# ethanabrooks/hsr-env

Measured on NVIDIA B200. Metric: env_actions_per_sec, higher is better.
Workload: dtype f32

## Files before the change

### hsr_env_b200/csrc/hsr_core.h

```cpp
#pragma once
#include <cfloat>
#include <cmath>
#include <cstdint>

#include "hsr_model.h"

#if defined(__CUDACC__)
#define HSR_HD __host__ __device__ __forceinline__
#define HSR_HDN __host__ __device__ __noinline__
#if defined(HSR_COMPACT)
#define HSR_HDC __host__ __device__ __noinline__
#else
#define HSR_HDC __host__ __device__ __forceinline__
#endif
#else
#define HSR_HDC inline
#define HSR_HD inline
#define HSR_HDN inline
#endif

#if defined(HSR_SCAN_NOISE) && !defined(__CUDA_ARCH__)
static thread_local unsigned long long hsr_scan_noise_seed = 0;
#endif

// ... 489 lines not shown
  st3(r, cross(va, fa) + cross(vl, fl)); st3(r + 3, cross(va, fl));
}

template <typename T>
HSR_HDC void smooth_lane0(const ModelT<T>& m, WS<T>& w) {
  int nv = m.nv;
  T (*cvel)[6] = reinterpret_cast<T(*)[6]>(w.cvel);
  T (*cacc)[6] = reinterpret_cast<T(*)[6]>(w.cacc);
  T (*cfrc)[6] = reinterpret_cast<T(*)[6]>(w.cfrc);
  for (int k = 0; k < 6; k++) { cvel[0][k] = 0; cacc[0][k] = 0; cfrc[0][k] = 0; }
  cacc[0][3] = -m.gravity[0]; cacc[0][4] = -m.gravity[1]; cacc[0][5] = -m.gravity[2];
  for (int b = 1; b < m.nbody; b++) {
    int p = m.body_parent[b];
    T v[6], a[6], t[6];
    for (int k = 0; k < 6; k++) { v[k] = cvel[p][k]; a[k] = cacc[p][k]; }
    for (int j = m.body_jntadr[b]; j < m.body_jntadr[b] + m.body_jntnum[b]; j++) {
      int d0 = m.jnt_dofadr[j];
      if (m.jnt_type[j] == JNT_FREE) {
        for (int k = 0; k < 3; k++) for (int i = 0; i < 6; i++) v[i] += w.cdof[6 * (d0 + k) + i] * w.qvel[d0 + k];
        T vt[6];
        for (int i = 0; i < 6; i++) vt[i] = v[i];
        for (int k = 3; k < 6; k++) {
          cross_motion(vt, w.cdof + 6 * (d0 + k), t);
          for (int i = 0; i < 6; i++) { a[i] += t[i] * w.qvel[d0 + k]; v[i] += w.cdof[6 * (d0 + k) + i] * w.qvel[d0 + k]; }
        }
      } else {
        cross_motion(v, w.cdof + 6 * d0, t);
        for (int i = 0; i < 6; i++) { a[i] += t[i] * w.qvel[d0]; v[i] += w.cdof[6 * d0 + i] * w.qvel[d0]; }
      }
    }
    T Ia[6], Iv[6];
    inert_mul(w.binert + 10 * b, a, Ia);
    inert_mul(w.binert + 10 * b, v, Iv);
    cross_force(v, Iv, t);
    for (int k = 0; k < 6; k++) { cvel[b][k] = v[k]; cacc[b][k] = a[k]; cfrc[b][k] = Ia[k] + t[k]; }
  }
  for (int b = m.nbody - 1; b > 0; b--) {
    int p = m.body_parent[b];
    if (p > 0) for (int k = 0; k < 6; k++) cfrc[p][k] += cfrc[b][k];
  }
  for (int i = 0; i < nv; i++) {
    const T* c = w.cdof + 6 * i;
    const T* f = cfrc[m.dof_body[i]];
    T bias = c[0] * f[0] + c[1] * f[1] + c[2] * f[2] + c[3] * f[3] + c[4] * f[4] + c[5] * f[5];
    w.qfrc_smooth[i] = -m.dof_damping[i] * w.qvel[i] - bias;
  }
  for (int a = 0; a < m.nu; a++) {
    T c = w.ctrl[a];
    if (m.act_ctrllimited[a]) c = fmin(fmax(c, m.act_ctrlrange[2 * a]), m.act_ctrlrange[2 * a + 1]);
    T f = m.act_kp[a] * c - m.act_kp[a] * m.act_gear[a] * w.qpos[m.act_qposadr[a]];
    if (m.act_forcelimited[a]) f = fmin(fmax(f, m.act_forcerange[2 * a]), m.act_forcerange[2 * a + 1]);
    w.qfrc_smooth[m.act_dof[a]] += m.act_gear[a] * f;
  }
}
template <typename T, typename Grp>
HSR_HD void smooth_solve(const ModelT<T>& m, WS<T>& w, const Grp& g) {
  const int nv = m.nv;
  for (int k = g.lane; k < nv * nv; k += Grp::G) w.L[k] = w.M[k];
  for (int i = g.lane; i < nv; i += Grp::G) w.qacc_smooth[i] = w.qfrc_smooth[i];
  g.sync();
  if (!chol_factor_g(w.L, nv, w.invd, g) && g.lane == 0) w.wi[WI_FLAGS] |= FLAG_CHOL;
  chol_solve_g(w.L, nv, w.invd, w.qacc_smooth, g);
}

template <typename T> struct Geom {
  int type; T size[3]; const T* verts; int nvert; V3<GT> pos; GT mat[9];
  const T* verts4 = nullptr;
};

template <typename T>
HSR_HD void load_geom(const ModelT<T>& m, const WS<T>& w, int gi, Geom<T>& ge) {
  ge.type = m.geom_type[gi];
  for (int k = 0; k < 3; k++) ge.size[k] = m.geom_size[3 * gi + k];
  ge.verts = m.hull_vert + 3 * m.geom_vertadr[gi]; ge.nvert = m.geom_vertnum[gi];
  ge.pos = ld3(w.gpos + 3 * gi);
  GT gm[9];
  for (int k = 0; k < 9; k++) gm[k] = (GT)m.geom_mat[9 * gi + k];
  mulm(w.xmat + 9 * m.geom_body[gi], gm, ge.mat);
}

template <typename T> HSR_HD void make_frame(V3<GT> n, T* fr) {
  n = normalized(n);
  V3<GT> t = (n.y > GT(-0.5) && n.y < GT(0.5)) ? mk<GT>(0, 1, 0) : mk<GT>(0, 0, 1);
  t = t - n * dot(n, t);
  t = normalized(t);
  st3c(fr, n); st3c(fr + 3, t); st3c(fr + 6, cross(n, t));
}

template <typename T, typename Grp>
HSR_HDC void add_contact(const ModelT<T>& m, WS<T>& w, const Grp& g, int& ncon, int& nrow, int pair, GT dist, V3<GT> pos,
                        V3<GT> n) {
  int dim = m.pair_condim[pair];
  if (ncon >= m.ncon_max || nrow + dim > m.nefc_max) {
    if (g.lane == 0) w.wi[WI_FLAGS] |= FLAG_CON_OVERFLOW;
    return;
  }
  if (g.lane == 0) {
    w.con_pair[ncon] = pair; w.con_dist[ncon] = (T)dist; st3c(w.con_pos + 3 * ncon, pos);
    make_frame(n, w.con_frame + 9 * ncon);
    w.con_adr[ncon] = nrow;
  }
  ncon++; nrow += dim;
}

template <typename T> struct Sup { V3<T> v, v1, v2; };

template <typename T> HSR_HD bool is_zero(T x) { return fabs(x) < Lim<T>::eps(); }
template <typename T> HSR_HD bool ccd_eq(T a, T b) {
  T ab = fabs(a - b);
  if (ab < Lim<T>::eps()) return true;
  a = fabs(a); b = fabs(b);
  return ab < Lim<T>::eps() * (b > a ? b : a);
}

template <typename T> HSR_HD T origin_tri_dist2(V3<T> a, V3<T> b, V3<T> c, V3<T>& q) {
  V3<T> ab = b - a, ac = c - a, ap = -a;
  T d1 = dot(ab, ap), d2 = dot(ac, ap);
  if (d1 <= 0 && d2 <= 0) { q = a; return dot(q, q); }
  V3<T> bp = -b;
  T d3 = dot(ab, bp), d4 = dot(ac, bp);
  if (d3 >= 0 && d4 <= d3) { q = b; return dot(q, q); }
  T vc = d1 * d4 - d3 * d2;
  V3<T> cp = -c;
  T d5 = dot(ab, cp), d6 = dot(ac, cp);
  if (vc <= 0 && d1 >= 0 && d3 <= 0) { q = a + ab * (d1 / (d1 - d3)); return dot(q, q); }
  if (d6 >= 0 && d5 <= d6) { q = c; return dot(q, q); }
  T vb = d5 * d2 - d1 * d6, va = d3 * d6 - d5 * d4;
  if (vb <= 0 && d2 >= 0 && d6 <= 0) { q = a + ac * (d2 / (d2 - d6)); return dot(q, q); }
  if (va <= 0 && (d4 - d3) >= 0 && (d5 - d6) >= 0) { q = b + (c - b) * ((d4 - d3) / ((d4 - d3) + (d5 - d6))); return dot(q, q); }
  T den = T(1) / (va + vb + vc);
  q = a + ab * (vb * den) + ac * (vc * den);
  return dot(q, q);
}

#define HSR_SUPPORT_TIE 1e-12
template <typename T> HSR_HD T scan_slack(T best) { return sizeof(T) == 4 ? T(1e-6) * (T(1) + fabs(best)) : T(HSR_SUPPORT_TIE); }
HSR_HD double dot3_exact(double x, double y, double z, double lx, double ly, double lz) {
#if defined(__CUDA_ARCH__)
  return __dadd_rn(__dadd_rn(__dmul_rn(x, lx), __dmul_rn(y, ly)), __dmul_rn(z, lz));
#else
  volatile double a = x * lx, b = y * ly, c = z * lz;
  volatile double ab = a + b;
  return ab + c;
#endif
}

template <typename T> HSR_HD void load_vert(const T* p, int st, T& x, T& y, T& z) { (void)st; x = p[0]; y = p[1]; z = p[2]; }
#if defined(__CUDACC__)
template <> HSR_HD void load_vert<float>(const float* p, int st, float& x, float& y, float& z) {
  if (st == 4) { const float4 a = *reinterpret_cast<const float4*>(p); x = a.x; y = a.y; z = a.z; }
  else { x = p[0]; y = p[1]; z = p[2]; }
}
#endif
template <typename T, typename Grp>
HSR_HD int hull_argmax(const T* __restrict__ v, int st, int n, V3<double> dl, const Grp& g) {
  const T lx = (T)dl.x, ly = (T)dl.y, lz = (T)dl.z;
  T best = -FLT_MAX, second = -FLT_MAX;
  int bi = 0x7fffffff;
  for (int i = g.lane; i < n; i += Grp::G) {
    T px, py, pz;
    load_vert(v + (size_t)st * i, st, px, py, pz);
    T val = px * lx + py * ly + pz * lz;
#if defined(HSR_SCAN_NOISE) && !defined(__CUDA_ARCH__)
    if (hsr_scan_noise_seed) {
      hsr_scan_noise_seed = hsr_scan_noise_seed * 6364136223846793005ull + 1442695040888963407ull;
      val += (T)(fabs((double)val) * 2.4e-7 * ((double)(hsr_scan_noise_seed >> 40) / 16777216.0 - 0.5));
    }
#endif
    if (val > best) bi = i;
    second = fmax(second, fmin(best, val));
    best = fmax(best, val);
  }
  T gbest = best;
  int gbi = bi;
  g.argmax(gbest, gbi);
  const T cut = gbest - scan_slack(gbest);
  const unsigned involved = g.ballot(best >= cut);
  const unsigned multi = g.ballot(second >= cut);
  if (multi == 0 && (involved & (involved - 1)) == 0) return gbi;
  if (multi == 0) {
    double dv = -DBL_MAX;
    if (best >= cut) {
      T px, py, pz;
      load_vert(v + (size_t)st * bi, st, px, py, pz);
      dv = dot3_exact((double)px, (double)py, (double)pz, dl.x, dl.y, dl.z);
    }
    const double dmax = g.max(dv);
    return g.min(dv >= dmax - HSR_SUPPORT_TIE ? bi : 0x7fffffff);
  }
  double dbest = -DBL_MAX;
  if (best >= cut) {
    for (int i = g.lane; i < n; i += Grp::G) {
      T px, py, pz;
      load_vert(v + (size_t)st * i, st, px, py, pz);
      const T val = px * lx + py * ly + pz * lz;
      if (val >= cut) { const double d = dot3_exact((double)px, (double)py, (double)pz, dl.x, dl.y, dl.z); if (d > dbest) dbest = d; }
    }
  }
  dbest = g.max(dbest);
  int mi = 0x7fffffff;
  if (best >= cut) {
    for (int i = g.lane; i < n; i += Grp::G) {
      T px, py, pz;
      load_vert(v + (size_t)st * i, st, px, py, pz);
      const T val = px * lx + py * ly + pz * lz;
      if (val >= cut && i < mi && dot3_exact((double)px, (double)py, (double)pz, dl.x, dl.y, dl.z) >= dbest - HSR_SUPPORT_TIE) mi = i;
    }
  }
  return g.min(mi);
}

template <typename T, typename Grp>
HSR_HD V3<double> support_d(const Geom<T>& ge, V3<double> d, const Grp& g) {
  typedef double W;
  const W* R = ge.mat;
  V3<W> dl = multv(R, d), res;
  const W tie = -HSR_SUPPORT_TIE;
  if (ge.type == GEOM_BOX) {
    res = mk<W>(dl.x >= tie ? (W)ge.size[0] : -(W)ge.size[0], dl.y >= tie ? (W)ge.size[1] : -(W)ge.size[1],
                dl.z >= tie ? (W)ge.size[2] : -(W)ge.size[2]);
  } else if (ge.type == GEOM_CYLINDER) {
    W n = sqrt(dl.x * dl.x + dl.y * dl.y);
    res = mk<W>(0, 0, dl.z >= tie ? (W)ge.size[1] : -(W)ge.size[1]);
    if (n > 1e-15) { res.x = dl.x / n * (W)ge.size[0]; res.y = dl.y / n * (W)ge.size[0]; }
#if defined(__CUDACC__)
  } else if (ge.verts4) {
    const int bi = hull_argmax<float>(ge.verts4, 4, ge.nvert, dl, g);
    res = mk<W>((W)ge.verts4[4 * bi], (W)ge.verts4[4 * bi + 1], (W)ge.verts4[4 * bi + 2]);
#endif
  } else {
    const int bi = hull_argmax<T>(ge.verts, 3, ge.nvert, dl, g);
    res = mk<W>((W)ge.verts[3 * bi], (W)ge.verts[3 * bi + 1], (W)ge.verts[3 * bi + 2]);
  }
  return ge.pos + mulv(R, res);
}

template <typename T, typename Grp>
HSR_HD void mpr_support(const Geom<T>& g1, const Geom<T>& g2, V3<double> d, const Grp& g, Sup<double>& s) {
  s.v1 = support_d(g1, d, g); s.v2 = support_d(g2, -d, g); s.v = s.v1 - s.v2;
}

template <typename T, typename Grp>
HSR_HD bool mpr_penetration_inl(const Geom<T>& g1, const Geom<T>& g2, GT tol, int max_iter, const Grp& g, GT& depth_,
                                V3<GT>& pdir_, V3<GT>& ppos_, float* sep = nullptr);
template <typename T, typename Grp>
HSR_HDN bool mpr_penetration(const Geom<T>& g1, const Geom<T>& g2, GT tol, int max_iter, const Grp& g, GT& depth_,
                             V3<GT>& pdir_, V3<GT>& ppos_, float* sep = nullptr) {
  return mpr_penetration_inl(g1, g2, tol, max_iter, g, depth_, pdir_, ppos_, sep);
}
template <typename T, typename Grp>
HSR_HD bool mpr_penetration_inl(const Geom<T>& g1, const Geom<T>& g2, GT tol, int max_iter, const Grp& g, GT& depth_,
                                V3<GT>& pdir_, V3<GT>& ppos_, float* sep) {
  typedef double W;
  auto sup = [&](V3<W> d) { Sup<W> s; mpr_support(g1, g2, d, g, s); return s; };
  auto miss = [&](V3<W> d) {
    if (sep && g.lane == 0) { sep[0] = (float)d.x; sep[1] = (float)d.y; sep[2] = (float)d.z; sep[3] = 1.f; }
    return false;
  };
  if (sep && sep[3] == 1.f) {
    V3<W> dc = normalized(mk<W>((W)sep[0], (W)sep[1], (W)sep[2]));
    Sup<W> sc = sup(dc);
    W dtc = dot(sc.v, dc);
    if (dtc < 0 && !is_zero(dtc)) return false;
    g.sync();
    if (g.lane == 0) sep[3] = 0.f;
  }
  auto reach_tol = [&](const Sup<W>& v1, const Sup<W>& v2, const Sup<W>& v3, const Sup<W>& v4, V3<W> d) {
    W dv4 = dot(v4.v, d);
    W d1 = dv4 - dot(v1.v, d), d2 = dv4 - dot(v2.v, d), d3 = dv4 - dot(v3.v, d);
    W mn = fmin(d1, fmin(d2, d3));
    return ccd_eq(mn, tol) || mn < tol;
  };
  auto expand = [&](const Sup<W>& v0, Sup<W>& v1, Sup<W>& v2, Sup<W>& v3, const Sup<W>& v4) {
    V3<W> v4v0 = cross(v4.v, v0.v);
    if (dot(v1.v, v4v0) > 0) {
      if (dot(v2.v, v4v0) > 0) v1 = v4; else v3 = v4;
    } else {
      if (dot(v3.v, v4v0) > 0) v2 = v4; else v1 = v4;
    }
  };
  auto finish = [&](W depth, V3<W> dir, V3<W> pos) {
    depth_ = depth; pdir_ = dir; ppos_ = pos;
    if (sep && g.lane == 0) sep[3] = 2.f;
    return true;
  };
  const W eps = Lim<W>::eps();
  Sup<W> v0, v1, v2, v3, v4;
  v0.v1 = g1.pos; v0.v2 = g2.pos;
  v0.v = v0.v1 - v0.v2;
  if (fabs(v0.v.x) < eps && fabs(v0.v.y) < eps && fabs(v0.v.z) < eps) v0.v.x += eps * 10;
  V3<W> d = normalized(-v0.v);
  v1 = sup(d);
  W dt = dot(v1.v, d);
  if (is_zero(dt) || dt < 0) return dt < 0 && !is_zero(dt) ? miss(d) : false;
  d = cross(v0.v, v1.v);
  if (is_zero(dot(d, d))) {
    if (fabs(v1.v.x) < eps && fabs(v1.v.y) < eps && fabs(v1.v.z) < eps) return false;
    W dep = norm(v1.v);
    return finish(dep, v1.v * (W(1) / dep), (v1.v1 + v1.v2) * W(0.5));
  }
  d = normalized(d);
  v2 = sup(d);
  dt = dot(v2.v, d);
  if (is_zero(dt) || dt < 0) return dt < 0 && !is_zero(dt) ? miss(d) : false;
  d = normalized(cross(v1.v - v0.v, v2.v - v0.v));
  if (dot(d, v0.v) > 0) { Sup<W> t = v1; v1 = v2; v2 = t; d = -d; }
  for (int guard = 0; guard < 64; guard++) {
    v3 = sup(d);
    dt = dot(v3.v, d);
    if (is_zero(dt) || dt < 0) return dt < 0 && !is_zero(dt) ? miss(d) : false;
    bool cont = false;
    dt = dot(cross(v1.v, v3.v), v0.v);
    if (dt < 0 && !is_zero(dt)) { v2 = v3; cont = true; }
    if (!cont) {
      dt = dot(cross(v3.v, v2.v), v0.v);
      if (dt < 0 && !is_zero(dt)) { v1 = v3; cont = true; }
    }
    if (!cont) break;
    d = normalized(cross(v1.v - v0.v, v2.v - v0.v));
  }
  for (int guard = 0; guard < 256; guard++) {
    d = normalized(cross(v2.v - v1.v, v3.v - v1.v));
    dt = dot(d, v1.v);
    if (is_zero(dt) || dt > 0) break;
    v4 = sup(d);
    dt = dot(v4.v, d);
    if (!(is_zero(dt) || dt > 0)) return miss(d);
    if (reach_tol(v1, v2, v3, v4, d)) return false;
    expand(v0, v1, v2, v3, v4);
  }
  int it = 0;
  while (true) {
    d = normalized(cross(v2.v - v1.v, v3.v - v1.v));
    v4 = sup(d);
    if (reach_tol(v1, v2, v3, v4, d) || it > max_iter) {
      V3<W> q;
      W d2 = origin_tri_dist2(v1.v, v2.v, v3.v, q);
      W dep = sqrt(d2);
      if (is_zero(dep)) return false;
      V3<W> dir = q * (W(1) / norm(q));
      W b0 = dot(cross(v1.v, v2.v), v3.v), b1 = dot(cross(v3.v, v2.v), v0.v), b2 = dot(cross(v0.v, v1.v), v3.v),
        b3 = dot(cross(v2.v, v1.v), v0.v);
      W s = b0 + b1 + b2 + b3;
      if (is_zero(s) || s < 0) {
        b0 = 0; b1 = dot(cross(v2.v, v3.v), d); b2 = dot(cross(v3.v, v1.v), d); b3 = dot(cross(v1.v, v2.v), d);
        s = b1 + b2 + b3;
      }
      W inv = W(1) / s;
      V3<W> p1 = (v0.v1 * b0 + v1.v1 * b1 + v2.v1 * b2 + v3.v1 * b3) * inv;
      V3<W> p2 = (v0.v2 * b0 + v1.v2 * b1 + v2.v2 * b2 + v3.v2 * b3) * inv;
      return finish(dep, dir, (p1 + p2) * W(0.5));
    }
    expand(v0, v1, v2, v3, v4);
    it++;
  }
}

template <typename T, typename Grp>
HSR_HDN void box_box(const ModelT<T>& m, WS<T>& w, const Grp& g, int& ncon, int& nrow, int pair, const Geom<T>& A,
                     const Geom<T>& B) {
  const GT* R1 = A.mat; const GT* R2 = B.mat;
  const GT s1[3] = {(GT)A.size[0], (GT)A.size[1], (GT)A.size[2]}, s2[3] = {(GT)B.size[0], (GT)B.size[1], (GT)B.size[2]};
// ... 876 lines not shown
```

### hsr_env_b200/csrc/hsrb_wpe.cuh

```cuda
#pragma once
#include "hsrb_push.cuh"

#ifndef WPE_MAXCON
#define WPE_MAXCON 8
#endif
#define WPE_GROUPS (WPE_MAXCON + 2)
#define WPE_SLOTS (6 * WPE_GROUPS)
#define WPE_MAXROW (6 * WPE_MAXCON + 2)
#define WPE_MAXBG 2
#define WPE_MAXGEOM 24
#define WPE_MAXPAIR 24
#define WPE_ENVJOBS 7
#ifndef WPE_MAXWARPS
#define WPE_MAXWARPS 28
#endif

namespace wpe {

struct alignas(16) Tab {
  double gbase[WPE_MAXGEOM * 3];
  double gmatw[WPE_MAXGEOM * 9];
  double pairc[WPE_MAXPAIR * PUSH_PAIRC];
  float ghalf[WPE_MAXGEOM * 3];
  float geom_rbound[WPE_MAXGEOM];
  float geom_size[WPE_MAXGEOM * 3];
  float pair_friction[WPE_MAXPAIR * 5];
  float bgeom_mat[WPE_MAXBG * 9];
  float geom_aabb[WPE_MAXGEOM * 3];
  int gmove[WPE_MAXGEOM], geom_type[WPE_MAXGEOM], geom_vertadr[WPE_MAXGEOM], geom_vertnum[WPE_MAXGEOM];
  int pair_geom1[WPE_MAXPAIR], pair_geom2[WPE_MAXPAIR], pair_func[WPE_MAXPAIR], pair_condim[WPE_MAXPAIR];
  float pair_sr[WPE_MAXPAIR], pair_sb[WPE_MAXPAIR];
  int gb0;
  float blk_radius;
  int wpt;
  unsigned char team[WPE_MAXWARPS];
};

struct alignas(16) Slice {
  double xb[4], Rb[10], bmat[9 * WPE_MAXBG], gpos[WPE_MAXGEOM * 3], portal[48], mres[8];
  float qpos[12], qvel[8], warm[8], mocap[4], ctrl[4];
  float baabb[4 * WPE_MAXBG];
  float qs[8], as[8], x[8], qfc[8], srch[8];
  float con_dist[WPE_MAXCON], con_pos[WPE_MAXCON * 3], con_frame[WPE_MAXCON * 9];
  int con_pair[WPE_MAXCON], con_adr[WPE_MAXCON], wi[4];
  int acc[8];
  float jres[WPE_ENVJOBS * 14 + 2];
  float J[WPE_SLOTS * 8];
  float Dr[WPE_SLOTS], aref[WPE_SLOTS], rsc[WPE_SLOTS], jar[WPE_SLOTS], jv[WPE_SLOTS], f[WPE_SLOTS], wrow[WPE_SLOTS];
  float PQ[16 * WPE_GROUPS], wpq[2 * WPE_GROUPS + 4], L[64];
  float sep[4 * WPE_MAXPAIR];
};

#define WPE_MAXTEAMS 4
struct alignas(16) Queue {
  int cnt[WPE_MAXTEAMS][4];
  int jobs[WPE_MAXWARPS * WPE_ENVJOBS];
};

static_assert(offsetof(Slice, J) % 16 == 0 && offsetof(Slice, PQ) % 16 == 0 && offsetof(Slice, L) % 16 == 0 && offsetof(Slice, qpos) % 16 == 0 &&
              offsetof(Slice, qvel) % 16 == 0 && offsetof(Slice, qs) % 16 == 0 && offsetof(Slice, x) % 16 == 0 && offsetof(Slice, srch) % 16 == 0 &&
              offsetof(Slice, warm) % 16 == 0 && offsetof(Slice, as) % 16 == 0 && sizeof(Slice) % 16 == 0,
              "128-bit shared-memory accesses (push::ld8 / st8) need 16-byte aligned fields");
__host__ __device__ inline size_t slice_bytes() { return sizeof(Slice); }
constexpr unsigned SMEM_HEAD = (unsigned)(sizeof(Tab) + sizeof(Queue));
static_assert(SMEM_HEAD % 16 == 0, "the slices start 16-byte aligned");
__host__ __device__ inline size_t shared_tail(const ModelT<float>& m) { return SMEM_HEAD + (size_t)m.nvert * 16 + 16; }

}

#if defined(HSRB_WPE_IMPL)
namespace wpe {

typedef V3<double> V3d;

__device__ __forceinline__ unsigned char* smem_base() {
  HSRB_DYN_SMEM(smem);
  return smem;
}
__device__ __forceinline__ Tab& tab() { return *reinterpret_cast<Tab*>(smem_base()); }
__device__ __forceinline__ Queue& queue() { return *reinterpret_cast<Queue*>(smem_base() + sizeof(Tab)); }
__device__ __forceinline__ Slice& slice(int w) { return *reinterpret_cast<Slice*>(smem_base() + SMEM_HEAD + (unsigned)w * (unsigned)sizeof(Slice)); }
__device__ __forceinline__ float* hull_verts4() {
  return reinterpret_cast<float*>(smem_base() + SMEM_HEAD + (blockDim.x >> 5) * (unsigned)sizeof(Slice));
}

#if defined(WPE_CHAIN_CLOCKS)
__device__ unsigned long long wpe_ck_cyc[32], wpe_ck_cnt[32];
#define WPE_CK_DECL long long ck_last = clock64()
#define WPE_CK_RESET() do { ck_last = clock64(); } while (0)
#define WPE_CK(id) do { if ((threadIdx.x & 31) == 0) { const long long t_ = clock64(); atomicAdd(&wpe::wpe_ck_cyc[id], (unsigned long long)(t_ - ck_last)); atomicAdd(&wpe::wpe_ck_cnt[id], 1ull); } ck_last = clock64(); } while (0)
#else
#define WPE_CK_DECL do { } while (0)
#define WPE_CK_RESET() do { } while (0)
#define WPE_CK(id) do { } while (0)
#endif

#if defined(HSRB_SIMT_EMU)
__device__ __forceinline__ void team_sync(int team, int nthreads) { emu::named_barrier(1 + team, nthreads); }
__device__ __forceinline__ bool team_and(int team, int nthreads, bool p) { return emu::named_vote(1 + team, nthreads, p, true); }
#else
__device__ __forceinline__ void team_sync(int team, int nthreads) {
  asm volatile("bar.sync %0, %1;" ::"r"(1 + team), "r"(nthreads) : "memory");
}
__device__ __forceinline__ bool team_and(int team, int nthreads, bool p) {
  unsigned r;
  asm volatile(
      "{\n\t.reg .pred q, r;\n\tsetp.ne.u32 q, %3, 0;\n\tbar.red.and.pred r, %1, %2, q;\n\tselp.u32 %0, 1, 0, r;\n\t}"
      : "=r"(r) : "r"(1 + team), "r"(nthreads), "r"((unsigned)p) : "memory");
  return r != 0;
}
#endif

__device__ __forceinline__ float warp_sum(float v) {
#pragma unroll
  for (int o = 16; o > 0; o >>= 1) v += __shfl_xor_sync(0xffffffffu, v, o);
  return v;
}

__device__ __forceinline__ const double* geom_mat(const Tab& t, const Slice& s, int gi, int gb0) {
  return t.gmove[gi] == 2 ? s.bmat + 9 * (gi - gb0) : t.gmatw + 9 * gi;
}

#ifndef WPE_SUPPORT_ATTR
#define WPE_SUPPORT_ATTR __forceinline__
#endif
__device__ WPE_SUPPORT_ATTR V3d support(const Tab& t, const Slice& s, const float* verts4, int gi, int gb0, V3d d) {
  WPE_CK_DECL;
  const double* R = geom_mat(t, s, gi, gb0);
  const V3d dl = multv(R, d);
  const int type = t.geom_type[gi];
  const float* sz = t.geom_size + 3 * gi;
  V3d res;
  const double tie = -HSR_SUPPORT_TIE;
  if (type == GEOM_BOX) {
    res = mk<double>(dl.x >= tie ? (double)sz[0] : -(double)sz[0], dl.y >= tie ? (double)sz[1] : -(double)sz[1],
                     dl.z >= tie ? (double)sz[2] : -(double)sz[2]);
  } else if (type == GEOM_CYLINDER) {
    const double n = sqrt(dl.x * dl.x + dl.y * dl.y);
    res = mk<double>(0, 0, dl.z >= tie ? (double)sz[1] : -(double)sz[1]);
    if (n > 1e-15) { res.x = dl.x / n * (double)sz[0]; res.y = dl.y / n * (double)sz[0]; }
  } else {
    const DevGrp<32> gw;
    const float* v4 = verts4 + 4 * t.geom_vertadr[gi];
    WPE_CK(22);
    const int bi = hull_argmax<float>(v4, 4, t.geom_vertnum[gi], dl, gw);
    WPE_CK(23);
    res = mk<double>((double)v4[4 * bi], (double)v4[4 * bi + 1], (double)v4[4 * bi + 2]);
  }
  const V3d out_ = ld3(s.gpos + 3 * gi) + mulv(R, res);
  WPE_CK(type == GEOM_BOX ? 25 : 24);
  return out_;
}

__device__ __forceinline__ V3d pv(const Slice& s, int k) { return ld3(s.portal + 9 * k); }
__device__ __forceinline__ void pcopy(Slice& s, int dst, int src) {
  const int lane = threadIdx.x & 31;
  __syncwarp();
  if (lane < 9) s.portal[9 * dst + lane] = s.portal[9 * src + lane];
  __syncwarp();
}

__device__ __noinline__ bool mpr(int ow, int g1, int g2, int gb0, float tol_f, int max_iter, int sepk) {
  const Tab& t = tab();
  const Slice& o = slice(ow);
  Slice& s = slice(threadIdx.x >> 5);
  const float* const verts4 = hull_verts4();
  float* const sep = sepk >= 0 ? slice(ow).sep + 4 * sepk : nullptr;
  const double tol = (double)tol_f;
  double* const out7 = s.mres;
  double* const P = s.portal;
  const int lane = threadIdx.x & 31;
  enum { S_CACHE = 0, S_V1, S_V2, S_DISCOVER, S_REFINE, S_PENETRATE };
  const double eps = DBL_EPSILON;
  int state = S_V1;
  V3d dcur;
  {
    V3d v0 = ld3(o.gpos + 3 * g1) - ld3(o.gpos + 3 * g2);
    if (fabs(v0.x) < eps && fabs(v0.y) < eps && fabs(v0.z) < eps) v0.x += eps * 10;
    V3d d;
    if (sep && (sep[3] == 1.f || sep[3] < 0.f)) {
      state = S_CACHE;
      d = normalized(mk<double>((double)sep[0], (double)sep[1], (double)sep[2]));
    } else {
      d = normalized(-v0);
    }
    __syncwarp();
    if (lane == 0) { st3(P, v0); st3(P + 3, ld3(o.gpos + 3 * g1)); st3(P + 6, ld3(o.gpos + 3 * g2)); }
    __syncwarp();
    dcur = d;
  }
  int guard = 0, it = 0;
  WPE_CK_DECL;
#define WPE_NEXT_DIR() { dcur = d; WPE_CK(21); continue; }
#pragma unroll 1
  while (true) {
    const V3d a1 = support(t, o, verts4, g1, gb0, dcur);
    const V3d a2 = support(t, o, verts4, g2, gb0, -dcur);
    const V3d v4 = a1 - a2;
    __syncwarp();
    if (lane == 0) { st3(P + 36, v4); st3(P + 39, a1); st3(P + 42, a2); }
    WPE_CK(20);
    V3d d = dcur;
    const V3d v0 = ld3(P);
    double dt = dot(v4, d);
    bool enter_refine = false;
    if (state == S_CACHE) {
      if (dt < 0 && !is_zero(dt)) {
        if (lane == 0) sep[3] = (float)(dt * 0.999);
        return false;
      }
      if (lane == 0) sep[3] = 0.f;
      state = S_V1;
      d = normalized(-v0);
      WPE_NEXT_DIR();
    }
    if (state <= S_DISCOVER) {
      if (is_zero(dt) || dt < 0) {
        if (dt < 0 && !is_zero(dt) && sep && lane == 0) { sep[0] = (float)d.x; sep[1] = (float)d.y; sep[2] = (float)d.z; sep[3] = (float)(dt * 0.999); }
        return false;
      }
    }
    if (state == S_V1) {
      pcopy(s, 1, 4);
      d = cross(v0, v4);
      if (is_zero(dot(d, d))) {
        if (fabs(v4.x) < eps && fabs(v4.y) < eps && fabs(v4.z) < eps) return false;
        const double dep = norm(v4);
        const V3d dir = v4 * (1.0 / dep), pos = (a1 + a2) * 0.5;
        if (lane == 0) {
          out7[0] = dep; out7[1] = dir.x; out7[2] = dir.y; out7[3] = dir.z; out7[4] = pos.x; out7[5] = pos.y; out7[6] = pos.z;
          if (sep) sep[3] = 2.f;
        }
        __syncwarp();
        return true;
      }
      d = normalized(d);
      state = S_V2;
      WPE_NEXT_DIR();
    }
    if (state == S_V2) {
      pcopy(s, 2, 4);
      const V3d v1 = pv(s, 1);
      d = normalized(cross(v1 - v0, v4 - v0));
      if (dot(d, v0) > 0) {
        pcopy(s, 2, 1); pcopy(s, 1, 4);
        d = -d;
      }
      state = S_DISCOVER; guard = 0;
      WPE_NEXT_DIR();
    }
    if (state == S_DISCOVER) {
      pcopy(s, 3, 4);
      const V3d v1 = pv(s, 1), v2 = pv(s, 2);
      bool cont = false;
      dt = dot(cross(v1, v4), v0);
      if (dt < 0 && !is_zero(dt)) { pcopy(s, 2, 3); cont = true; }
      if (!cont) {
        dt = dot(cross(v4, v2), v0);
        if (dt < 0 && !is_zero(dt)) { pcopy(s, 1, 3); cont = true; }
      }
      guard++;
      if (cont && guard < 64) {
        const V3d w1 = pv(s, 1), w2 = pv(s, 2);
        d = normalized(cross(w1 - v0, w2 - v0));
        WPE_NEXT_DIR();
      }
      state = S_REFINE; guard = 0;
      enter_refine = true;
    }
    if (state == S_REFINE && !enter_refine) {
      if (!(is_zero(dt) || dt > 0)) {
        if (sep && lane == 0) { sep[0] = (float)d.x; sep[1] = (float)d.y; sep[2] = (float)d.z; sep[3] = (float)(dt * 0.999); }
        return false;
      }
    }
    if (state == S_PENETRATE || (state == S_REFINE && !enter_refine)) {
      const V3d v1 = pv(s, 1), v2 = pv(s, 2), v3 = pv(s, 3);
      const double d1 = dt - dot(v1, d), d2 = dt - dot(v2, d), d3 = dt - dot(v3, d);
      const double mn = fmin(d1, fmin(d2, d3));
      const bool reach = ccd_eq(mn, tol) || mn < tol;
      if (state == S_REFINE) {
        if (reach) return false;
      } else if (reach || it > max_iter) {
        V3d q;
        const double dd2 = origin_tri_dist2(v1, v2, v3, q);
        const double dep = sqrt(dd2);
        if (is_zero(dep)) return false;
        const V3d dir = q * (1.0 / norm(q));
        double b0 = dot(cross(v1, v2), v3), b1 = dot(cross(v3, v2), v0), b2 = dot(cross(v0, v1), v3), b3 = dot(cross(v2, v1), v0);
        double sm = b0 + b1 + b2 + b3;
        if (is_zero(sm) || sm < 0) {
          b0 = 0; b1 = dot(cross(v2, v3), d); b2 = dot(cross(v3, v1), d); b3 = dot(cross(v1, v2), d);
          sm = b1 + b2 + b3;
        }
        const double inv = 1.0 / sm;
        const double* P = s.portal;
        const V3d p1 = (ld3(P + 3) * b0 + ld3(P + 12) * b1 + ld3(P + 21) * b2 + ld3(P + 30) * b3) * inv;
        const V3d p2 = (ld3(P + 6) * b0 + ld3(P + 15) * b1 + ld3(P + 24) * b2 + ld3(P + 33) * b3) * inv;
        const V3d pos = (p1 + p2) * 0.5;
        if (lane == 0) {
          out7[0] = dep; out7[1] = dir.x; out7[2] = dir.y; out7[3] = dir.z; out7[4] = pos.x; out7[5] = pos.y; out7[6] = pos.z;
          if (sep) sep[3] = 2.f;
        }
        __syncwarp();
        return true;
      }
      const V3d v4v0 = cross(v4, v0);
      int repl;
      if (dot(v1, v4v0) > 0) repl = dot(v2, v4v0) > 0 ? 1 : 3;
      else repl = dot(v3, v4v0) > 0 ? 2 : 1;
      pcopy(s, repl, 4);
      if (state == S_REFINE) guard++; else it++;
    }
    {
      const V3d v1 = pv(s, 1), v2 = pv(s, 2), v3 = pv(s, 3);
      d = normalized(cross(v2 - v1, v3 - v1));
      if (state == S_REFINE) {
        const double dv = dot(d, v1);
        if (is_zero(dv) || dv > 0 || guard >= 256) state = S_PENETRATE;
      }
    }
    WPE_NEXT_DIR();
  }
#undef WPE_NEXT_DIR
}

__device__ __forceinline__ int* team_jobs(Queue& Q, const Tab& t, int w) { return Q.jobs + t.team[w] * t.wpt * WPE_ENVJOBS; }

}

#if defined(HSRB_PHASE_CLOCKS)
#define WPE_PH(id) do { if (LOCK && threadIdx.x == 0) { const long long t_ = clock64(); ph[id] += (unsigned long long)(t_ - tlast) >> 4; tlast = t_; } } while (0)
#else
#define WPE_PH(id) do { } while (0)
#endif
template <bool LOCK>
__global__ void __launch_bounds__(32 * WPE_MAXWARPS, 1) hsrb_wpe_kernel_t(const __grid_constant__ KArgs a, const __grid_constant__ PushInfo fi) {
  constexpr unsigned FULL = 0xffffffffu;
  const int lane = threadIdx.x & 31, wib = threadIdx.x >> 5, wpb = blockDim.x >> 5;
  const ModelT<float>& m = a.m;
  wpe::Tab& tw = wpe::tab();
  wpe::Queue& Q = wpe::queue();
  float* const v4w = wpe::hull_verts4();
  {
    const int ng = m.ngeom, np = m.npair;
    for (int i = threadIdx.x; i < m.nvert * 4; i += blockDim.x) v4w[i] = fi.verts4[i];
#define TAB_COPY(field, src, n) for (int i = threadIdx.x; i < (n); i += blockDim.x) tw.field[i] = (src)[i];
    TAB_COPY(gbase, fi.gbase, ng * 3) TAB_COPY(gmatw, fi.gmatw, ng * 9) TAB_COPY(pairc, fi.pairc, np * PUSH_PAIRC)
    TAB_COPY(ghalf, fi.ghalf, ng * 3) TAB_COPY(geom_rbound, m.geom_rbound, ng)
    TAB_COPY(geom_size, m.geom_size, ng * 3) TAB_COPY(pair_friction, m.pair_friction, np * 5)
    TAB_COPY(geom_aabb, m.geom_aabb, ng * 3)
    {
      int gb0_ = ng;
      for (int i = ng - 1; i >= 0; i--) if (fi.gmove[i] == 2) gb0_ = i;
      for (int i = threadIdx.x; i < (ng - gb0_) * 9 && i < WPE_MAXBG * 9; i += blockDim.x) tw.bgeom_mat[i] = m.geom_mat[9 * gb0_ + i];
      if (threadIdx.x == 0) {
        float blk_radius = 0.f;
        for (int i = gb0_; i < ng; i++) {
          const double* o3 = fi.gbase + 3 * i;
          blk_radius = fmaxf(blk_radius, (float)sqrt(o3[0] * o3[0] + o3[1] * o3[1] + o3[2] * o3[2]) * 1.001f + m.geom_rbound[i]);
        }
        tw.gb0 = gb0_; tw.blk_radius = blk_radius;
      }
      int nteam = LOCK ? (int)((a.opts >> 4) & 15u) : 1;
      if (nteam < 1 || nteam > WPE_MAXTEAMS || wpb % nteam != 0) nteam = 1;
      if (threadIdx.x == 0) tw.wpt = wpb / nteam;
      if (threadIdx.x < wpb) tw.team[threadIdx.x] = (unsigned char)(threadIdx.x / (wpb / nteam));
    }
    TAB_COPY(gmove, fi.gmove, ng) TAB_COPY(geom_type, m.geom_type, ng)
    TAB_COPY(geom_vertadr, m.geom_vertadr, ng) TAB_COPY(geom_vertnum, m.geom_vertnum, ng)
    TAB_COPY(pair_geom1, m.pair_geom1, np) TAB_COPY(pair_geom2, m.pair_geom2, np)
    TAB_COPY(pair_func, m.pair_func, np) TAB_COPY(pair_condim, m.pair_condim, np)
#undef TAB_COPY
    for (int k = threadIdx.x; k < np; k += blockDim.x) {
      const int b1 = m.geom_body[m.pair_geom1[k]], b2 = m.geom_body[m.pair_geom2[k]];
      tw.pair_sr[k] = (float)(b2 == fi.robot_body) - (float)(b1 == fi.robot_body);
      tw.pair_sb[k] = (float)(b2 == fi.block_body) - (float)(b1 == fi.block_body);
    }
    if (threadIdx.x < 4 * WPE_MAXTEAMS) (&Q.cnt[0][0])[threadIdx.x] = 0;
    __syncthreads();
  }
  const wpe::Tab& t = tw;
  const float* const verts4 = v4w;
  wpe::Slice& s = wpe::slice(wib);
  const int NV = fi.nv;
  const bool HASB = NV == 8;
  const int nq = m.nq;
  const float dt = m.timestep;
  const int li = lane & 7, sub = lane >> 3;
  const float scale = 1.0f / (m.meaninertia * (float)(NV > 1 ? NV : 1));
  const float Mi = li < NV ? fi.Mdiag[li] : 1.0f, dampi = li < NV ? fi.damp[li] : 0.f;
  const bool use_sep = !(a.opts & 1u);
  const bool use_gap = use_sep && !(a.opts & 0x10000u);
#if !defined(HSRB_SIMT_EMU)
  if (LOCK && t.team[wib] > 0 && ((a.opts >> 8) & 255u)) {
    const long long t0 = clock64(), wait = (long long)((a.opts >> 8) & 255u) * 4 * 1965 * t.team[wib];
    while (clock64() - t0 < wait) __nanosleep(1000);
  }
#endif
#if defined(WPE_DEBUG_JOBS)
  long long dbg_long = 0, dbg_quick = 0; int dbg_nlong = 0, dbg_nquick = 0, dbg_hits = 0, dbg_jobs_total = 0, dbg_long_total = 0, dbg_sub = 0;
#endif
#if defined(HSRB_PHASE_CLOCKS)
  unsigned long long ph[PH_COUNT] = {0, 0, 0, 0, 0, 0, 0};
  long long tlast = clock64();
#endif

#pragma unroll 1
  for (int wave0 = 0; wave0 < a.n; wave0 += gridDim.x * wpb) {
    const int slot = wave0 + wib * (int)gridDim.x + (int)blockIdx.x;
    const bool valid = slot < a.n;
    const int env = valid ? (a.order ? a.order[slot] : slot) : 0;
    if (!LOCK && !valid) break;
    if (valid) {
      const float* st = a.state + (size_t)env * a.S;
      if (lane < 12) s.qpos[lane] = (lane < nq) ? st[lane] : 0.f;
      if (lane < 8) {
        s.qvel[lane] = lane < NV ? st[nq + lane] : 0.f;
        s.warm[lane] = lane < NV ? st[nq + NV + lane] : 0.f;
        s.qfc[lane] = 0.f;
      }
      if (lane < 3) s.mocap[lane] = st[nq + 2 * NV + lane];
      if (lane < 2) s.ctrl[lane] = (a.ctrl && lane < fi.act_n) ? a.ctrl[(size_t)env * m.nu + lane] : 0.f;
      if (lane < 4) s.wi[lane] = 0;
      for (int i = lane; i < 4 * m.npair; i += 32) s.sep[i] = 0.f;
      for (int i = lane; i < m.ngeom * 3; i += 32) s.gpos[i] = t.gbase[i];
      if (lane < 3) s.xb[lane] = 0;
      if (lane < 9) s.Rb[lane] = (lane % 4 == 0) ? 1.0 : 0.0;
    }
    int flags = 0;
    enum { A_ITER = 0, A_LS, A_CON, A_EFC, A_KFLOP, A_NARROW, A_HIT };
    if (lane < 8) s.acc[lane] = 0;
#if defined(WPE_CHAIN_CLOCKS)
    const long long ck_env0 = clock64();
#endif
    bool success = false;
    int taken = 0;
    bool finished = !valid || a.nsub <= 0;
    __syncwarp();

#pragma unroll 1
    for (int sb_ = 0; sb_ < a.nsub; sb_++) {
      if (LOCK) { if (wpe::team_and(t.team[wib], 32 * t.wpt, finished)) break; }
      else if (finished) break;
#if defined(HSRB_PHASE_CLOCKS)
      if (LOCK && threadIdx.x == 0) tlast = clock64();
#endif
      int nlimit = 0, ncon = 0, nefc = 0, narrow = 0, npflop = 0, ngrp = 0, nslot = 0, gdim = 0, nskip = 0;
      unsigned bits = 0;
      int it = 0, ls_used = 0;
      WPE_CK_DECL;
      if (!finished) {
      if (HASB) {
        double qd[4] = {(double)s.qpos[5], (double)s.qpos[6], (double)s.qpos[7], (double)s.qpos[8]};
        quatnormalize(qd);
        double Rb[9];
        quat2mat(qd, Rb);
        __syncwarp();
        if (lane < 4) s.qpos[5 + lane] = (float)qd[lane];
        if (lane < 3) s.xb[lane] = (double)s.qpos[2 + lane];
        if (lane == 0) {
#pragma unroll
          for (int k = 0; k < 9; k++) s.Rb[k] = Rb[k];
        }
// ... 791 lines not shown
```

Baseline: 216,600.

## Unroll hull support scan and keep MPR portal candidate in registers

Splits hull_argmax into a scan phase and a pick phase. The scan can now keep U independent running maxima so vertex loads can overlap, with U set to 2 for the warp-per-env path. The MPR portal's candidate point (v4, a1, a2) is no longer written to shared slot 4. Each of lanes 0-8 holds one component in a register and writes it straight into its destination slot, which shrinks the shared Slice portal array and removes a store plus a sync. The sep pointer becomes a lazily evaluated lambda, and the extra unrolled accumulators cost registers.

```diff
diff --git a/hsr_env_b200/csrc/hsr_core.h b/hsr_env_b200/csrc/hsr_core.h
--- a/hsr_env_b200/csrc/hsr_core.h
+++ b/hsr_env_b200/csrc/hsr_core.h
@@ -665,25 +665,47 @@
   else { x = p[0]; y = p[1]; z = p[2]; }
 }
 #endif
-template <typename T, typename Grp>
-HSR_HD int hull_argmax(const T* __restrict__ v, int st, int n, V3<double> dl, const Grp& g) {
+template <typename T> struct HullScan { T best, second; int bi; };
+template <int U, typename T, typename Grp>
+HSR_HD HullScan<T> hull_scan(const T* __restrict__ v, int st, int n, V3<double> dl, const Grp& g) {
   const T lx = (T)dl.x, ly = (T)dl.y, lz = (T)dl.z;
-  T best = -FLT_MAX, second = -FLT_MAX;
-  int bi = 0x7fffffff;
-  for (int i = g.lane; i < n; i += Grp::G) {
-    T px, py, pz;
-    load_vert(v + (size_t)st * i, st, px, py, pz);
-    T val = px * lx + py * ly + pz * lz;
+  HullScan<T> a[U];
+#pragma unroll
+  for (int u = 0; u < U; u++) { a[u].best = -FLT_MAX; a[u].second = -FLT_MAX; a[u].bi = 0x7fffffff; }
+  for (int i0 = g.lane; i0 < n; i0 += U * Grp::G) {
+#pragma unroll
+    for (int u = 0; u < U; u++) {
+      const int i = i0 + u * Grp::G;
+      const bool in = u == 0 || i < n;
+      T px, py, pz;
+      load_vert(v + (size_t)st * (in ? i : i0), st, px, py, pz);
+      T val = px * lx + py * ly + pz * lz;
 #if defined(HSR_SCAN_NOISE) && !defined(__CUDA_ARCH__)
-    if (hsr_scan_noise_seed) {
-      hsr_scan_noise_seed = hsr_scan_noise_seed * 6364136223846793005ull + 1442695040888963407ull;
-      val += (T)(fabs((double)val) * 2.4e-7 * ((double)(hsr_scan_noise_seed >> 40) / 16777216.0 - 0.5));
-    }
+      if (hsr_scan_noise_seed && in) {
+        hsr_scan_noise_seed = hsr_scan_noise_seed * 6364136223846793005ull + 1442695040888963407ull;
+        val += (T)(fabs((double)val) * 2.4e-7 * ((double)(hsr_scan_noise_seed >> 40) / 16777216.0 - 0.5));
+      }
 #endif
-    if (val > best) bi = i;
-    second = fmax(second, fmin(best, val));
-    best = fmax(best, val);
-  }
+      if (!in) val = -FLT_MAX;
+      if (val > a[u].best) a[u].bi = i;
+      a[u].second = fmax(a[u].second, fmin(a[u].best, val));
+      a[u].best = fmax(a[u].best, val);
+    }
+  }
+#pragma unroll
+  for (int u = 1; u < U; u++) {
+    if (a[u].best > a[0].best || (a[u].best == a[0].best && a[u].bi < a[0].bi)) a[0].bi = a[u].bi;
+    a[0].second = fmax(fmax(a[0].second, a[u].second), fmin(a[0].best, a[u].best));
+    a[0].best = fmax(a[0].best, a[u].best);
+  }
+  return a[0];
+}
+
+template <typename T, typename Grp>
+HSR_HD int hull_pick(const T* __restrict__ v, int st, int n, V3<double> dl, const Grp& g, const HullScan<T>& sc) {
+  const T lx = (T)dl.x, ly = (T)dl.y, lz = (T)dl.z;
+  const T best = sc.best, second = sc.second;
+  const int bi = sc.bi;
   T gbest = best;
   int gbi = bi;
   g.argmax(gbest, gbi);
@@ -721,6 +743,11 @@
     }
   }
   return g.min(mi);
+}
+
+template <typename T, typename Grp>
+HSR_HD int hull_argmax(const T* __restrict__ v, int st, int n, V3<double> dl, const Grp& g) {
+  return hull_pick(v, st, n, dl, g, hull_scan<1>(v, st, n, dl, g));
 }
 
 template <typename T, typename Grp>
diff --git a/hsr_env_b200/csrc/hsrb_wpe.cuh b/hsr_env_b200/csrc/hsrb_wpe.cuh
--- a/hsr_env_b200/csrc/hsrb_wpe.cuh
+++ b/hsr_env_b200/csrc/hsrb_wpe.cuh
@@ -37,7 +37,7 @@
 };
 
 struct alignas(16) Slice {
-  double xb[4], Rb[10], bmat[9 * WPE_MAXBG], gpos[WPE_MAXGEOM * 3], portal[48], mres[8];
+  double xb[4], Rb[10], bmat[9 * WPE_MAXBG], gpos[WPE_MAXGEOM * 3], portal[36], mres[8];
   float qpos[12], qvel[8], warm[8], mocap[4], ctrl[4];
   float baabb[4 * WPE_MAXBG];
   float qs[8], as[8], x[8], qfc[8], srch[8];
@@ -121,6 +121,9 @@
   return t.gmove[gi] == 2 ? s.bmat + 9 * (gi - gb0) : t.gmatw + 9 * gi;
 }
 
+#ifndef WPE_SCAN_U
+#define WPE_SCAN_U 2
+#endif
 #ifndef WPE_SUPPORT_ATTR
 #define WPE_SUPPORT_ATTR __forceinline__
 #endif
@@ -142,8 +145,9 @@
   } else {
     const DevGrp<32> gw;
     const float* v4 = verts4 + 4 * t.geom_vertadr[gi];
+    const int nv = t.geom_vertnum[gi];
     WPE_CK(22);
-    const int bi = hull_argmax<float>(v4, 4, t.geom_vertnum[gi], dl, gw);
+    const int bi = hull_pick<float>(v4, 4, nv, dl, gw, hull_scan<WPE_SCAN_U>(v4, 4, nv, dl, gw));
     WPE_CK(23);
     res = mk<double>((double)v4[4 * bi], (double)v4[4 * bi + 1], (double)v4[4 * bi + 2]);
   }
@@ -153,6 +157,20 @@
 }
 
 __device__ __forceinline__ V3d pv(const Slice& s, int k) { return ld3(s.portal + 9 * k); }
+__device__ __forceinline__ double pvpart(V3d v, V3d a1, V3d a2) {
+  const int lane = threadIdx.x & 31;
+  double x = v.x;
+  x = lane == 1 ? v.y : x; x = lane == 2 ? v.z : x;
+  x = lane == 3 ? a1.x : x; x = lane == 4 ? a1.y : x; x = lane == 5 ? a1.z : x;
+  x = lane == 6 ? a2.x : x; x = lane == 7 ? a2.y : x; x = lane == 8 ? a2.z : x;
+  return x;
+}
+__device__ __forceinline__ void pset(Slice& s, int dst, double x) {
+  const int lane = threadIdx.x & 31;
+  __syncwarp();
+  if (lane < 9) s.portal[9 * dst + lane] = x;
+  __syncwarp();
+}
 __device__ __forceinline__ void pcopy(Slice& s, int dst, int src) {
   const int lane = threadIdx.x & 31;
   __syncwarp();
@@ -165,7 +183,8 @@
   const Slice& o = slice(ow);
   Slice& s = slice(threadIdx.x >> 5);
   const float* const verts4 = hull_verts4();
-  float* const sep = sepk >= 0 ? slice(ow).sep + 4 * sepk : nullptr;
+  const bool has_sep = sepk >= 0;
+  const auto sep = [&]() { return slice(ow).sep + 4 * sepk; };
   const double tol = (double)tol_f;
   double* const out7 = s.mres;
   double* const P = s.portal;
@@ -178,9 +197,9 @@
     V3d v0 = ld3(o.gpos + 3 * g1) - ld3(o.gpos + 3 * g2);
     if (fabs(v0.x) < eps && fabs(v0.y) < eps && fabs(v0.z) < eps) v0.x += eps * 10;
     V3d d;
-    if (sep && (sep[3] == 1.f || sep[3] < 0.f)) {
+    if (has_sep && (sep()[3] == 1.f || sep()[3] < 0.f)) {
       state = S_CACHE;
-      d = normalized(mk<double>((double)sep[0], (double)sep[1], (double)sep[2]));
+      d = normalized(mk<double>((double)sep()[0], (double)sep()[1], (double)sep()[2]));
     } else {
       d = normalized(-v0);
     }
@@ -197,8 +216,7 @@
     const V3d a1 = support(t, o, verts4, g1, gb0, dcur);
     const V3d a2 = support(t, o, verts4, g2, gb0, -dcur);
     const V3d v4 = a1 - a2;
-    __syncwarp();
-    if (lane == 0) { st3(P + 36, v4); st3(P + 39, a1); st3(P + 42, a2); }
+    const double x4 = pvpart(v4, a1, a2);
     WPE_CK(20);
     V3d d = dcur;
     const V3d v0 = ld3(P);
@@ -206,22 +224,22 @@
     bool enter_refine = false;
     if (state == S_CACHE) {
       if (dt < 0 && !is_zero(dt)) {
-        if (lane == 0) sep[3] = (float)(dt * 0.999);
+        if (lane == 0) sep()[3] = (float)(dt * 0.999);
         return false;
       }
-      if (lane == 0) sep[3] = 0.f;
+      if (lane == 0) sep()[3] = 0.f;
       state = S_V1;
       d = normalized(-v0);
       WPE_NEXT_DIR();
     }
     if (state <= S_DISCOVER) {
       if (is_zero(dt) || dt < 0) {
-        if (dt < 0 && !is_zero(dt) && sep && lane == 0) { sep[0] = (float)d.x; sep[1] = (float)d.y; sep[2] = (float)d.z; sep[3] = (float)(dt * 0.999); }
+        if (dt < 0 && !is_zero(dt) && has_sep && lane == 0) { sep()[0] = (float)d.x; sep()[1] = (float)d.y; sep()[2] = (float)d.z; sep()[3] = (float)(dt * 0.999); }
         return false;
       }
     }
     if (state == S_V1) {
-      pcopy(s, 1, 4);
+      pset(s, 1, x4);
       d = cross(v0, v4);
       if (is_zero(dot(d, d))) {
         if (fabs(v4.x) < eps && fabs(v4.y) < eps && fabs(v4.z) < eps) return false;
@@ -229,7 +247,7 @@
         const V3d dir = v4 * (1.0 / dep), pos = (a1 + a2) * 0.5;
         if (lane == 0) {
           out7[0] = dep; out7[1] = dir.x; out7[2] = dir.y; out7[3] = dir.z; out7[4] = pos.x; out7[5] = pos.y; out7[6] = pos.z;
-          if (sep) sep[3] = 2.f;
+          if (has_sep) sep()[3] = 2.f;
         }
         __syncwarp();
         return true;
@@ -239,18 +257,18 @@
       WPE_NEXT_DIR();
     }
     if (state == S_V2) {
-      pcopy(s, 2, 4);
+      pset(s, 2, x4);
       const V3d v1 = pv(s, 1);
       d = normalized(cross(v1 - v0, v4 - v0));
       if (dot(d, v0) > 0) {
-        pcopy(s, 2, 1); pcopy(s, 1, 4);
+        pcopy(s, 2, 1); pset(s, 1, x4);
         d = -d;
       }
       state = S_DISCOVER; guard = 0;
       WPE_NEXT_DIR();
     }
     if (state == S_DISCOVER) {
-      pcopy(s, 3, 4);
+      pset(s, 3, x4);
       const V3d v1 = pv(s, 1), v2 = pv(s, 2);
       bool cont = false;
       dt = dot(cross(v1, v4), v0);
@@ -270,7 +288,7 @@
     }
     if (state == S_REFINE && !enter_refine) {
       if (!(is_zero(dt) || dt > 0)) {
-        if (sep && lane == 0) { sep[0] = (float)d.x; sep[1] = (float)d.y; sep[2] = (float)d.z; sep[3] = (float)(dt * 0.999); }
+        if (has_sep && lane == 0) { sep()[0] = (float)d.x; sep()[1] = (float)d.y; sep()[2] = (float)d.z; sep()[3] = (float)(dt * 0.999); }
         return false;
       }
     }
@@ -300,7 +318,7 @@
         const V3d pos = (p1 + p2) * 0.5;
         if (lane == 0) {
           out7[0] = dep; out7[1] = dir.x; out7[2] = dir.y; out7[3] = dir.z; out7[4] = pos.x; out7[5] = pos.y; out7[6] = pos.z;
-          if (sep) sep[3] = 2.f;
+          if (has_sep) sep()[3] = 2.f;
         }
         __syncwarp();
         return true;
@@ -309,7 +327,7 @@
       int repl;
       if (dot(v1, v4v0) > 0) repl = dot(v2, v4v0) > 0 ? 1 : 3;
       else repl = dot(v3, v4v0) > 0 ? 2 : 1;
-      pcopy(s, repl, 4);
+      pset(s, repl, x4);
       if (state == S_REFINE) guard++; else it++;
     }
     {
```

Result: faster. 218,900 (median of 6 runs) (+1.1%).
